# opendilab/LightZero

Hardware: NVIDIA H100
Metric: MCTS simulations/sec (batched search+infer) (higher is better)
Workload: dtype f32 (fp16x2-split tensor MMAs, fp32 accumulate)

## Files before the change

### lightzero_b200/csrc/conv_tc.cu

```cuda
#include <math.h>
#include <stdlib.h>
#include <string.h>

#include <algorithm>

#include "conv_tc.cuh"
#include "tc_ptx.cuh"

namespace lz {

constexpr int kCvConsumers = 256, kCvThreads = kCvConsumers + 32;
constexpr int kCvStages = 4;

struct CvBars {
    uint64_t full[kCvStages], empty[kCvStages];
    uint64_t in_full;
};

struct CvGeom {
    int nbands, rin, m_lo, mcount, NT, PR;
    size_t plane, part, phase, in_bytes, tap_bytes, smem;
};

__host__ __device__ inline CvGeom cv_geom(const ConvTc &p)
{
    CvGeom g;
    const int H = p.in.H, pitch = p.in.pitch, kg = p.in.C / 8;
    g.nbands = (H + p.band_h - 1) / p.band_h;
    g.rin = (p.band_h + 2) * pitch + 2;
    g.m_lo = pitch + 1;
    g.mcount = (p.G - 1) * g.rin + p.band_h * pitch;
    g.NT = (g.mcount + 127) / 128;
    g.PR = g.m_lo + g.NT * 128 + pitch + 2;
    if (g.PR < p.G * g.rin) g.PR = p.G * g.rin;
    g.plane = (size_t)g.PR * 16;
    g.part = (size_t)kg * g.plane;
    g.phase = 2 * g.part;
    g.in_bytes = (g.phase * p.in.nphase + 127) & ~(size_t)127;
    g.tap_bytes = (size_t)2 * kg * p.N * 16;
    g.smem = g.in_bytes + p.stages * g.tap_bytes + 1024;
    return g;
}

__device__ __forceinline__ void store_split2(unsigned char *hi_ptr, unsigned char *lo_ptr, float a, float b)
{
    a = fminf(fmaxf(a, -65504.0f), 65504.0f);
    b = fminf(fmaxf(b, -65504.0f), 65504.0f);
    const __half ha = __float2half_rn(a), hb = __float2half_rn(b);
    *reinterpret_cast<__half2 *>(hi_ptr) = __halves2half2(ha, hb);
    *reinterpret_cast<__half2 *>(lo_ptr) = __halves2half2(__float2half_rn(a - __half2float(ha)), __float2half_rn(b - __half2float(hb)));
}

template <int N>
__global__ void __launch_bounds__(kCvThreads, N == 128 ? 1 : 2) k_conv_tc(ConvTc p)
{
    extern __shared__ __align__(1024) unsigned char smem[];
    const CvGeom g = cv_geom(p);
    unsigned char *in_s = smem;
    unsigned char *ring = smem + g.in_bytes;
    CvBars *bars = reinterpret_cast<CvBars *>(ring + p.stages * g.tap_bytes);
    const int nstages = p.stages;
    const int tid = threadIdx.x, warp = __shfl_sync(0xffffffffu, tid >> 5, 0), lane = tid & 31;
    const int pitch = p.in.pitch, H = p.in.H, W = p.in.W, kg_in = p.in.C / 8;
    const int group = blockIdx.x / g.nbands, band = blockIdx.x - group * g.nbands;
    const int img0 = group * p.G, nimg = min(p.G, p.B - img0);
    const int y0 = band * p.band_h;
    const int rin0 = y0 * pitch - 1;
    const int npass = p.npass;

    if (tid == 0) {
        for (int i = 0; i < kCvStages; ++i) { mbar_init(&bars->full[i], 1); mbar_init(&bars->empty[i], kCvConsumers / 32); }
        mbar_init(&bars->in_full, 1);
        fence_mbar_init();
    }
    __syncthreads();

    if (warp == kCvConsumers / 32) {
        if (lane == 0) {
            const int grow0 = rin0 + 1;
            const int ncopy = min(g.rin, p.in.plane_rows - grow0);
            const uint32_t bytes = (uint32_t)ncopy * 16u;
            mbar_expect_tx(&bars->in_full, bytes * (uint32_t)(nimg * p.in.nphase * 2 * kg_in));
            for (int k = 0; k < nimg; ++k)
                for (int f = 0; f < p.in.nphase; ++f)
                    for (int part = 0; part < 2; ++part)
                        for (int kg = 0; kg < kg_in; ++kg) {
                            const unsigned char *src = p.in.base + (size_t)(img0 + k) * p.in.img_stride + f * p.in.phase_stride +
                                                       part * p.in.part_stride + ((size_t)kg * p.in.plane_rows + grow0) * 16;
                            unsigned char *dst = in_s + f * g.phase + part * g.part + kg * g.plane + (size_t)k * g.rin * 16;
                            bulk_g2s(dst, src, bytes, &bars->in_full);
                        }
            for (int n = 0; n < 9 * g.NT; ++n) {
                const int st = n % nstages, tap = n % 9;
                if (n >= nstages) mbar_wait(&bars->empty[st], ((n / nstages) - 1) & 1);
                mbar_expect_tx(&bars->full[st], (uint32_t)g.tap_bytes);
                bulk_g2s(ring + st * g.tap_bytes, p.w + (size_t)tap * g.tap_bytes, (uint32_t)g.tap_bytes, &bars->full[st]);
            }
        }
        return;
    }

    const int wg = warp >> 2;
    const uint32_t plane16 = (uint32_t)(g.plane >> 4);
    const uint64_t a_desc0 = make_desc(smem_u32(in_s), plane16, 8);
    const uint64_t b_desc0 = make_desc(smem_u32(ring), 2 * N, 8);
    const uint32_t b_lo16 = (uint32_t)N;
    const uint32_t a_lo16 = (uint32_t)(g.part >> 4);
    const int nks = kg_in / 2;
    const int yend = min(y0 + p.band_h, H);
    const int qc = 2 * (lane & 3);
    mbar_wait(&bars->in_full, 0);
    for (int t = 0; t < g.NT; ++t) {
        float acc[N / 2];
#pragma unroll
        for (int i = 0; i < N / 2; ++i) acc[i] = 0.0f;
        for (int tap = 0; tap < 9; ++tap) {
            const int n = t * 9 + tap, st = n % nstages;
            mbar_wait(&bars->full[st], (n / nstages) & 1);
            const uint64_t b0 = b_desc0 + (uint64_t)((st * g.tap_bytes) >> 4);
            const uint64_t a0 = a_desc0 + (uint64_t)((p.tap_phase[tap] * g.phase) >> 4) + (uint64_t)(g.m_lo + p.tap_shift[tap] + t * 128 + wg * 64);
            wg_fence();
            for (int ks = 0; ks < nks; ++ks) {
                wgmma_f16<N>(acc, a0 + ks * 2 * plane16, b0 + ks * 4 * N);
                if (npass == 3) {
                    wgmma_f16<N>(acc, a0 + ks * 2 * plane16, b0 + b_lo16 + ks * 4 * N);
                    wgmma_f16<N>(acc, a0 + a_lo16 + ks * 2 * plane16, b0 + ks * 4 * N);
                }
            }
            wg_commit();
            if (tap > 0) {
                wg_wait<1>();
                __syncwarp();
                if (lane == 0) mbar_arrive(&bars->empty[(n - 1) % nstages]);
            }
        }
        wg_wait<0>();
        __syncwarp();
        if (lane == 0) mbar_arrive(&bars->empty[(t * 9 + 8) % nstages]);

#pragma unroll
        for (int hr = 0; hr < 2; ++hr) {
            const int m = g.m_lo + t * 128 + wg * 64 + 16 * (warp & 3) + (lane >> 2) + 8 * hr;
            const int k = m / g.rin;
            const int rho = rin0 + (m - k * g.rin);
            const int yy = rho / pitch - 1, xx = rho - (yy + 1) * pitch;
            const bool in_band = (k < nimg) && (rho >= pitch) && (yy >= y0) && (yy < yend);
            const bool valid = in_band && (xx < W);
#pragma unroll
            for (int j = 0; j < N / 8; ++j) {
                const int col = 8 * j + qc;
                const int grp = (N == 128) ? (col >> 6) : 0;
                const int c = col - grp * 64;
                const Tcl &o = p.out[grp];
                const bool relu = p.relu[grp] != 0;
                float v0 = fmaf(acc[4 * j + 2 * hr], __ldg(p.scale + col), __ldg(p.shift + col));
                float v1 = fmaf(acc[4 * j + 2 * hr + 1], __ldg(p.scale + col + 1), __ldg(p.shift + col + 1));
                if (p.res.base && grp == 0 && valid) {
                    const unsigned char *rp = p.res.base + (size_t)(img0 + k) * p.res.img_stride +
                                              ((size_t)(c >> 3) * p.res.plane_rows + rho + 1) * 16 + (c & 7) * 2;
                    const float2 a = __half22float2(*reinterpret_cast<const __half2 *>(rp));
                    const float2 b = __half22float2(*reinterpret_cast<const __half2 *>(rp + p.res.part_stride));
                    v0 += a.x + b.x;
                    v1 += a.y + b.y;
                }
                v0 = valid ? (relu ? fmaxf(v0, 0.0f) : v0) : 0.0f;
                v1 = valid ? (relu ? fmaxf(v1, 0.0f) : v1) : 0.0f;
                if (in_band) {
                    unsigned char *op = o.base + (size_t)(img0 + k) * o.img_stride + ((size_t)(c >> 3) * o.plane_rows + rho + 1) * 16 + (c & 7) * 2;
                    store_split2(op, op + o.part_stride, v0, v1);
                }
            }
        }
    }
}

constexpr int kRbChunks = 16;

struct RbBars {
    uint64_t full[kCvStages], empty[kCvStages];
    uint64_t chunk[kRbChunks];
};

struct RbGeom {
    int nbands, S, m_lo, NT1, NT2, PR, nchunk;
    size_t plane, part, buf, tap_bytes, smem;
};

__host__ __device__ inline RbGeom rb_geom(const ResBlockTc &p)
{
    RbGeom g;
    const int H = p.in.H, pitch = p.in.pitch, kg = p.in.C / 8;
    g.nbands = (H + p.band_h - 1) / p.band_h;
    g.S = (p.band_h + 4) * pitch + 2;
    g.m_lo = pitch + 1;
    g.NT1 = ((p.G - 1) * g.S + (p.band_h + 2) * pitch + 127) / 128;
    g.NT2 = ((p.G - 1) * g.S + p.band_h * pitch + 127) / 128;
    g.PR = p.G * g.S;
    g.nchunk = (g.PR + 127) / 128;
    g.plane = (size_t)g.PR * 16;
    g.part = (size_t)kg * g.plane;
    g.buf = (2 * g.part + 127) & ~(size_t)127;
    g.tap_bytes = (size_t)2 * kg * p.in.C * 16;
    g.smem = 2 * g.buf + p.stages * g.tap_bytes + 1024;
    return g;
}

template <int N>
__device__ __forceinline__ void rb_tiles(float (&acc)[2][N / 2], bool two, uint64_t a_desc0, int row0, const ResBlockTc &p,
                                         const RbGeom &g, uint64_t b_desc0, RbBars *bars, int n0, int lane)
{
    const uint32_t plane16 = (uint32_t)(g.plane >> 4), a_lo16 = (uint32_t)(g.part >> 4), b_lo16 = (uint32_t)N;
    const int nstages = p.stages;
#pragma unroll
    for (int s = 0; s < 2; ++s)
#pragma unroll
        for (int i = 0; i < N / 2; ++i) acc[s][i] = 0.0f;
    for (int tap = 0; tap < 9; ++tap) {
        const int n = n0 + tap, st = n % nstages;
        mbar_wait(&bars->full[st], (n / nstages) & 1);
        const uint64_t b0 = b_desc0 + (uint64_t)((st * g.tap_bytes) >> 4);
        const uint64_t a0 = a_desc0 + (uint64_t)(row0 + p.tap_shift[tap]);
        wg_fence();
        for (int ks = 0; ks < N / 16; ++ks) {
#pragma unroll
            for (int s = 0; s < 2; ++s) {
                if (s == 1 && !two) break;
                const uint64_t as = a0 + s * 128 + ks * 2 * plane16;
                wgmma_f16<N>(acc[s], as, b0 + ks * 4 * N);
                if (p.npass == 3) {
                    wgmma_f16<N>(acc[s], as, b0 + b_lo16 + ks * 4 * N);
                    wgmma_f16<N>(acc[s], as + a_lo16, b0 + ks * 4 * N);
                }
            }
        }
        wg_commit();
        if (tap > 0) {
            wg_wait<1>();
            __syncwarp();
            if (lane == 0) mbar_arrive(&bars->empty[(n - 1) % nstages]);
        }
    }
    wg_wait<0>();
    __syncwarp();
    if (lane == 0) mbar_arrive(&bars->empty[(n0 + 8) % nstages]);
}

template <int N>
__global__ void __launch_bounds__(kCvThreads, 1) k_resblock_tc(ResBlockTc p)
{
    extern __shared__ __align__(1024) unsigned char smem[];
    const RbGeom g = rb_geom(p);
    unsigned char *in_s = smem, *mid_s = smem + g.buf, *ring = smem + 2 * g.buf;
    RbBars *bars = reinterpret_cast<RbBars *>(ring + p.stages * g.tap_bytes);
    const int nstages = p.stages;
    const int tid = threadIdx.x, warp = __shfl_sync(0xffffffffu, tid >> 5, 0), lane = tid & 31;
    const int pitch = p.in.pitch, H = p.in.H, W = p.in.W, kg_in = N / 8;
    const int group = blockIdx.x / g.nbands, band = blockIdx.x - group * g.nbands;
    const int img0 = group * p.G, nimg = min(p.G, p.B - img0);
    const int y0 = band * p.band_h;
    const int np1 = (g.NT1 + 1) / 2, ntaps = 9 * (np1 + (g.NT2 + 1) / 2);

    if (tid == 0) {
        for (int i = 0; i < kCvStages; ++i) { mbar_init(&bars->full[i], 1); mbar_init(&bars->empty[i], kCvConsumers / 32); }
        for (int c = 0; c < g.nchunk; ++c) mbar_init(&bars->chunk[c], 1);
        fence_mbar_init();
    }
    __syncthreads();

    if (warp == kCvConsumers / 32) {
        if (lane == 0) {
            auto load_tap = [&](int n) {
                const int st = n % nstages, tap = n % 9;
                if (n >= nstages) mbar_wait(&bars->empty[st], ((n / nstages) - 1) & 1);
                mbar_expect_tx(&bars->full[st], (uint32_t)g.tap_bytes);
                bulk_g2s(ring + st * g.tap_bytes, p.w[n >= 9 * np1] + (size_t)tap * g.tap_bytes, (uint32_t)g.tap_bytes, &bars->full[st]);
            };
            for (int n = 0; n < nstages; ++n) load_tap(n);
            const int g0 = (y0 - 1) * pitch;
            const int r0 = max(0, -g0), r1 = min(g.S, p.in.plane_rows - g0);
            for (int c = 0; c < g.nchunk; ++c) {
                uint32_t rows = 0;
                for (int k = 0; k < nimg; ++k) rows += (uint32_t)max(0, min(k * g.S + r1, c * 128 + 128) - max(k * g.S + r0, c * 128));
                mbar_expect_tx(&bars->chunk[c], rows * 16u * (uint32_t)(2 * kg_in));
                for (int k = 0; k < nimg; ++k) {
                    const int lo = max(k * g.S + r0, c * 128), hi = min(k * g.S + r1, c * 128 + 128);
                    if (hi <= lo) continue;
                    for (int part = 0; part < 2; ++part)
                        for (int kg = 0; kg < kg_in; ++kg) {
                            const unsigned char *src = p.in.base + (size_t)(img0 + k) * p.in.img_stride + part * p.in.part_stride +
                                                       ((size_t)kg * p.in.plane_rows + g0 + lo - k * g.S) * 16;
                            bulk_g2s(in_s + part * g.part + kg * g.plane + (size_t)lo * 16, src, (uint32_t)(hi - lo) * 16u, &bars->chunk[c]);
                        }
                }
            }
            for (int n = nstages; n < ntaps; ++n) load_tap(n);
        }
        return;
    }

    const int wg = warp >> 2;
    const uint32_t plane16 = (uint32_t)(g.plane >> 4);
    const uint64_t in_desc = make_desc(smem_u32(in_s), plane16, 8), mid_desc = make_desc(smem_u32(mid_s), plane16, 8);
    const uint64_t b_desc0 = make_desc(smem_u32(ring), 2 * N, 8);
    const int qc = 2 * (lane & 3);
    if (tid < 2 * kg_in) *reinterpret_cast<uint4 *>(mid_s + tid * g.plane) = make_uint4(0u, 0u, 0u, 0u);

    int ready = 0;
    for (int t = 0; t < g.NT1; t += 2) {
        const bool two = t + 1 < g.NT1;
        const int need = min(g.nchunk, (t * 128 + 256 + 2 * pitch + 1) / 128 + 1);
        for (; ready < need; ++ready) mbar_wait(&bars->chunk[ready], 0);
        float acc[2][N / 2];
        rb_tiles<N>(acc, two, in_desc, g.m_lo + t * 128 + wg * 64, p, g, b_desc0, bars, t / 2 * 9, lane);
#pragma unroll
        for (int e = 0; e < 4; ++e) {
            const int s = e >> 1, hr = e & 1;
            if (s == 1 && !two) break;
            const int m = g.m_lo + (t + s) * 128 + wg * 64 + 16 * (warp & 3) + (lane >> 2) + 8 * hr;
            const int i = m - pitch;
            const int k = m / g.S;
            const int rho = (y0 - 1) * pitch - 1 + (m - k * g.S);
            const int yy = rho / pitch - 1, xx = rho - (yy + 1) * pitch;
            const bool valid = (k < nimg) && (rho >= pitch) && (yy >= y0 - 1) && (yy <= y0 + p.band_h) && (yy < H) && (xx < W);
            if (i >= g.PR) continue;
#pragma unroll
            for (int j = 0; j < N / 8; ++j) {
                const int col = 8 * j + qc;
                float v0 = fmaf(acc[s][4 * j + 2 * hr], __ldg(p.scale[0] + col), __ldg(p.shift[0] + col));
                float v1 = fmaf(acc[s][4 * j + 2 * hr + 1], __ldg(p.scale[0] + col + 1), __ldg(p.shift[0] + col + 1));
                v0 = valid ? fmaxf(v0, 0.0f) : 0.0f;
                v1 = valid ? fmaxf(v1, 0.0f) : 0.0f;
                unsigned char *op = mid_s + (size_t)(col >> 3) * g.plane + (size_t)i * 16 + (col & 7) * 2;
                store_split2(op, op + g.part, v0, v1);
            }
        }
    }
    for (; ready < g.nchunk; ++ready) mbar_wait(&bars->chunk[ready], 0);
    fence_proxy_async();
    asm volatile("bar.sync 1, %0;\n" ::"n"(kCvConsumers) : "memory");

    const int yend = min(y0 + p.band_h, H);
    for (int t = 0; t < g.NT2; t += 2) {
        const bool two = t + 1 < g.NT2;
        float acc[2][N / 2];
        rb_tiles<N>(acc, two, mid_desc, g.m_lo + t * 128 + wg * 64, p, g, b_desc0, bars, (np1 + t / 2) * 9, lane);
#pragma unroll
        for (int e = 0; e < 4; ++e) {
            const int s = e >> 1, hr = e & 1;
            if (s == 1 && !two) break;
            const int m = g.m_lo + (t + s) * 128 + wg * 64 + 16 * (warp & 3) + (lane >> 2) + 8 * hr;
            const int k = m / g.S;
            const int rho = y0 * pitch - 1 + (m - k * g.S);
            const int yy = rho / pitch - 1, xx = rho - (yy + 1) * pitch;
            const bool in_band = (k < nimg) && (rho >= pitch) && (yy >= y0) && (yy < yend);
            const bool valid = in_band && (xx < W);
            const Tcl &o = p.out;
            size_t obase = 0;
            bool do_write = in_band;
            if (in_band) {
                if (o.nphase == 1) {
                    obase = (size_t)(img0 + k) * o.img_stride + (size_t)(rho + 1) * 16;
                } else if (valid) {
                    const int ph = (yy & 1) * 2 + (xx & 1);
                    const int rho2 = ((yy >> 1) + 1) * o.pitch + (xx >> 1);
                    obase = (size_t)(img0 + k) * o.img_stride + ph * o.phase_stride + (size_t)(rho2 + 1) * 16;
                } else {
                    do_write = false;
                }
            }
#pragma unroll
            for (int j = 0; j < N / 8; ++j) {
                const int col = 8 * j + qc;
                float v0 = fmaf(acc[s][4 * j + 2 * hr], __ldg(p.scale[1] + col), __ldg(p.shift[1] + col));
                float v1 = fmaf(acc[s][4 * j + 2 * hr + 1], __ldg(p.scale[1] + col + 1), __ldg(p.shift[1] + col + 1));
                if (valid) {
                    const unsigned char *rp = in_s + (size_t)(col >> 3) * g.plane + (size_t)(m + pitch) * 16 + (col & 7) * 2;
                    const float2 a = __half22float2(*reinterpret_cast<const __half2 *>(rp));
                    const float2 b = __half22float2(*reinterpret_cast<const __half2 *>(rp + g.part));
                    v0 += a.x + b.x;
                    v1 += a.y + b.y;
                }
                v0 = valid ? fmaxf(v0, 0.0f) : 0.0f;
                v1 = valid ? fmaxf(v1, 0.0f) : 0.0f;
                if (do_write) {
                    unsigned char *op = o.base + obase + (size_t)(col >> 3) * o.plane_rows * 16 + (col & 7) * 2;
                    store_split2(op, op + o.part_stride, v0, v1);
                }
            }
        }
    }
}

__device__ __forceinline__ void tcl_load8(const Tcl &t, int img, int kg, int rho, float (&v)[8])
{
    const unsigned char *pp = t.base + (size_t)img * t.img_stride + ((size_t)kg * t.plane_rows + rho + 1) * 16;
    const uint4 rh = __ldg(reinterpret_cast<const uint4 *>(pp));
    const uint4 rl = __ldg(reinterpret_cast<const uint4 *>(pp + t.part_stride));
    const __half2 *hh = reinterpret_cast<const __half2 *>(&rh), *hl = reinterpret_cast<const __half2 *>(&rl);
#pragma unroll
    for (int j = 0; j < 4; ++j) {
        const float2 a = __half22float2(hh[j]), b = __half22float2(hl[j]);
        v[2 * j] = a.x + b.x;
        v[2 * j + 1] = a.y + b.y;
    }
}

__global__ void k_pool_tcl(Tcl in, Tcl out, float *out_nchw, int B, int Hout)
{
    const int kgs = in.C / 8;
    const size_t n = (size_t)B * kgs * Hout * Hout;
    for (size_t i = blockIdx.x * (size_t)blockDim.x + threadIdx.x; i < n; i += (size_t)gridDim.x * blockDim.x) {
        const int xo = (int)(i % Hout), yo = (int)((i / Hout) % Hout);
        const int kg = (int)((i / ((size_t)Hout * Hout)) % kgs), img = (int)(i / ((size_t)Hout * Hout * kgs));
        float s[8];
#pragma unroll
        for (int j = 0; j < 8; ++j) s[j] = 0.0f;
#pragma unroll
        for (int ky = 0; ky < 3; ++ky) {
            const int yy = 2 * yo + ky - 1;
            if (yy < 0 || yy >= in.H) continue;
#pragma unroll
            for (int kx = 0; kx < 3; ++kx) {
                const int xx = 2 * xo + kx - 1;
                if (xx < 0 || xx >= in.W) continue;
                float v[8];
                tcl_load8(in, img, kg, (yy + 1) * in.pitch + xx, v);
#pragma unroll
                for (int j = 0; j < 8; ++j) s[j] += v[j];
            }
        }
#pragma unroll
        for (int j = 0; j < 8; ++j) s[j] = s[j] / 9.0f;
        if (out_nchw) {
#pragma unroll
            for (int j = 0; j < 8; ++j) out_nchw[((size_t)img * in.C + kg * 8 + j) * Hout * Hout + yo * Hout + xo] = s[j];
        } else {
            unsigned char *op = out.base + (size_t)img * out.img_stride + ((size_t)kg * out.plane_rows + (yo + 1) * out.pitch + xo + 1) * 16;
            store_split8(op, op + out.part_stride, s);
        }
    }
}

__global__ void k_tcl_to_nchw(Tcl in, float *out_nchw, int B)
{
    const int kgs = in.C / 8, H = in.H, W = in.W;
    const size_t n = (size_t)B * kgs * H * W;
    for (size_t i = blockIdx.x * (size_t)blockDim.x + threadIdx.x; i < n; i += (size_t)gridDim.x * blockDim.x) {
        const int x = (int)(i % W), y = (int)((i / W) % H);
        const int kg = (int)((i / ((size_t)W * H)) % kgs), img = (int)(i / ((size_t)W * H * kgs));
        float v[8];
        tcl_load8(in, img, kg, (y + 1) * in.pitch + x, v);
#pragma unroll
        for (int j = 0; j < 8; ++j) out_nchw[((size_t)img * in.C + kg * 8 + j) * H * W + y * W + x] = v[j];
    }
}

int conv_tc_prepare_launch()
{
    const int big = 227 * 1024;
    LZ_CUDA_CHECK(cudaFuncSetAttribute(k_conv_tc<64>, cudaFuncAttributeMaxDynamicSharedMemorySize, big));
    LZ_CUDA_CHECK(cudaFuncSetAttribute(k_conv_tc<128>, cudaFuncAttributeMaxDynamicSharedMemorySize, big));
    LZ_CUDA_CHECK(cudaFuncSetAttribute(k_resblock_tc<32>, cudaFuncAttributeMaxDynamicSharedMemorySize, big));
    LZ_CUDA_CHECK(cudaFuncSetAttribute(k_resblock_tc<64>, cudaFuncAttributeMaxDynamicSharedMemorySize, big));
    return LZ_OK;
}

int conv_tc_launch(const ConvTc &p, cudaStream_t s)
{
    const CvGeom g = cv_geom(p);
    LZ_REQUIRE(g.smem <= 227 * 1024, LZ_EINVAL, "conv_tc: band needs %zu B shared memory", g.smem);
    LZ_REQUIRE(g.tap_bytes <= 16384 && (p.in.C % 16) == 0, LZ_EINVAL, "conv_tc: unsupported channel counts");
    LZ_REQUIRE(p.out[0].nphase == 1 && (p.N < 128 || p.out[1].nphase == 1), LZ_EINVAL, "conv_tc: phase-split output is not supported");
    const int groups = (p.B + p.G - 1) / p.G;
    const int grid = groups * g.nbands;
    switch (p.N) {
        case 64: k_conv_tc<64><<<grid, kCvThreads, g.smem, s>>>(p); break;
        case 128: k_conv_tc<128><<<grid, kCvThreads, g.smem, s>>>(p); break;
        default: LZ_REQUIRE(false, LZ_EINVAL, "conv_tc: N must be 64 or 128");
    }
    LZ_KERNEL_CHECK();
    return LZ_OK;
}

int resblock_tc_plan(ResBlockTc &p)
{
    const int H = p.in.H, W = p.in.W;
    ResBlockTc q = p;
    double best = -1.0;
    for (int G = 1; G <= 4; ++G)
        for (int bh = (G > 1 ? H : 1); bh <= H; ++bh)
            for (int st = 2; st <= 4; st += 2) {
                q.G = G; q.band_h = bh; q.stages = st;
                const RbGeom g = rb_geom(q);
                if (g.smem > 227 * 1024 || g.nchunk > kRbChunks) continue;
                double score = (double)(2 * G * H * W) / ((double)g.nbands * (g.NT1 + g.NT2) * 128);
                score *= (st == 4) ? 1.0 : 0.97;
                if (score > best + 1e-9) { best = score; p.G = G; p.band_h = bh; p.stages = st; }
            }
    LZ_REQUIRE(best > 0.0, LZ_EINVAL, "resblock_tc: no band of a %dx%d, %d-channel block fits shared memory", H, W, p.in.C);
    return LZ_OK;
}

int resblock_tc_launch(const ResBlockTc &p, cudaStream_t s)
{
    const RbGeom g = rb_geom(p);
    LZ_REQUIRE(g.smem <= 227 * 1024 && g.nchunk <= kRbChunks, LZ_EINVAL, "resblock_tc: band needs %zu B shared memory", g.smem);
    LZ_REQUIRE(p.in.nphase == 1 && p.out.C == p.in.C, LZ_EINVAL, "resblock_tc: unsupported input / output layout");
    const int grid = (p.B + p.G - 1) / p.G * g.nbands;
    switch (p.in.C) {
        case 32: k_resblock_tc<32><<<grid, kCvThreads, g.smem, s>>>(p); break;
        case 64: k_resblock_tc<64><<<grid, kCvThreads, g.smem, s>>>(p); break;
        default: LZ_REQUIRE(false, LZ_EINVAL, "resblock_tc: channels must be 32 or 64");
    }
    LZ_KERNEL_CHECK();
    return LZ_OK;
}

size_t conv_tc_packed_bytes(int cin, int ncols) { return (size_t)9 * 2 * (cin / 8) * ncols * 16; }

float conv_tc_pack(const float *w, int cin, int cout, int ncols, int col0, unsigned char *dst)
{
    float mx = 0.0f;
    for (size_t i = 0; i < (size_t)cout * cin * 9; ++i) mx = std::max(mx, fabsf(w[i]));
    int e = 0;
    if (mx > 0.0f) frexpf(mx, &e);
    const float scale = ldexpf(1.0f, 13 - e);
    const size_t tap_halves = (size_t)2 * (cin / 8) * ncols * 8, part_halves = (size_t)ncols * 8;
    __half *h = reinterpret_cast<__half *>(dst);
    for (int t = 0; t < 9; ++t)
        for (int co = 0; co < cout; ++co)
            for (int ci = 0; ci < cin; ++ci) {
                const float sv = w[((size_t)co * cin + ci) * 9 + t] * scale;
                const __half hi = __float2half_rn(sv);
                const __half lo = __float2half_rn(sv - __half2float(hi));
                const size_t off = (size_t)t * tap_halves + ((size_t)(ci / 8) * 2 * ncols + col0 + co) * 8 + (ci % 8);
                h[off] = hi;
                h[off + part_halves] = lo;
            }
    return scale;
}

int pool_tcl_launch(const Tcl &in, const Tcl &out, int B, cudaStream_t s)
{
    const size_t n = (size_t)B * (in.C / 8) * out.H * out.W;
    k_pool_tcl<<<(int)std::min<size_t>((n + 255) / 256, kNumSMs * 32), 256, 0, s>>>(in, out, nullptr, B, out.H);
    LZ_KERNEL_CHECK();
    return LZ_OK;
}

int pool_tcl_to_nchw_launch(const Tcl &in, float *out, int B, int Hout, cudaStream_t s)
{
    const size_t n = (size_t)B * (in.C / 8) * Hout * Hout;
    Tcl dummy = in;
    k_pool_tcl<<<(int)std::min<size_t>((n + 255) / 256, kNumSMs * 32), 256, 0, s>>>(in, dummy, out, B, Hout);
    LZ_KERNEL_CHECK();
    return LZ_OK;
}

int tcl_to_nchw_launch(const Tcl &in, float *out, int B, cudaStream_t s)
{
    k_tcl_to_nchw<<<tcl_to_nchw_ctas(in, B), 256, 0, s>>>(in, out, B);
    LZ_KERNEL_CHECK();
    return LZ_OK;
}

int tcl_to_nchw_ctas(const Tcl &in, int B)
{
    const size_t n = (size_t)B * (in.C / 8) * in.H * in.W;
    return (int)std::min<size_t>((n + 255) / 256, kNumSMs * 32);
}

}
```

### lightzero_b200/csrc/tc_ptx.cuh

```cuda
#pragma once
#include <cuda_fp16.h>
#include <cuda_runtime.h>
#include <stdint.h>
#include <stdio.h>

namespace lz {

__device__ __forceinline__ uint32_t smem_u32(const void *p) { return (uint32_t)__cvta_generic_to_shared(p); }

__device__ __forceinline__ void mbar_init(uint64_t *bar, uint32_t count)
{
    asm volatile("mbarrier.init.shared::cta.b64 [%0], %1;\n" ::"r"(smem_u32(bar)), "r"(count));
}
__device__ __forceinline__ void mbar_arrive(uint64_t *bar)
{
    asm volatile("{\n\t.reg .b64 st;\n\tmbarrier.arrive.shared::cta.b64 st, [%0];\n\t}\n" ::"r"(smem_u32(bar)) : "memory");
}
__device__ __forceinline__ void mbar_expect_tx(uint64_t *bar, uint32_t bytes)
{
    asm volatile("{\n\t.reg .b64 st;\n\tmbarrier.arrive.expect_tx.shared::cta.b64 st, [%0], %1;\n\t}\n" ::"r"(smem_u32(bar)), "r"(bytes) : "memory");
}
__device__ __forceinline__ void mbar_wait(uint64_t *bar, uint32_t parity)
{
    const uint32_t a = smem_u32(bar);
    for (uint32_t it = 0; it < (1u << 28); ++it) {
        uint32_t ok;
        asm volatile("{\n\t.reg .pred p;\n\tmbarrier.try_wait.parity.shared::cta.b64 p, [%1], %2;\n\tselp.u32 %0, 1, 0, p;\n\t}\n"
                     : "=r"(ok) : "r"(a), "r"(parity) : "memory");
        if (ok) return;
    }
    asm volatile("trap;\n");
}
__device__ __forceinline__ void bulk_g2s(void *dst, const void *src, uint32_t bytes, uint64_t *bar)
{
    asm volatile("cp.async.bulk.shared::cluster.global.mbarrier::complete_tx::bytes [%0], [%1], %2, [%3];\n"
                 ::"r"(smem_u32(dst)), "l"(src), "r"(bytes), "r"(smem_u32(bar)) : "memory");
}
__device__ __forceinline__ void fence_proxy_async() { asm volatile("fence.proxy.async.shared::cta;\n" ::: "memory"); }
__device__ __forceinline__ void fence_mbar_init() { asm volatile("fence.mbarrier_init.release.cluster;\n" ::: "memory"); }

__device__ __forceinline__ void wg_fence() { asm volatile("wgmma.fence.sync.aligned;\n" ::: "memory"); }
__device__ __forceinline__ void wg_commit() { asm volatile("wgmma.commit_group.sync.aligned;\n" ::: "memory"); }
template <int N>
__device__ __forceinline__ void wg_wait() { asm volatile("wgmma.wait_group.sync.aligned %0;\n" ::"n"(N) : "memory"); }

template <int N>
__device__ __forceinline__ void wg_fence_acc(float (&d)[N])
{
#pragma unroll
    for (int i = 0; i < N; ++i) asm volatile("" : "+f"(d[i])::"memory");
}

#define LZ_WG_R8(o) "+f"(d[o + 0]), "+f"(d[o + 1]), "+f"(d[o + 2]), "+f"(d[o + 3]), "+f"(d[o + 4]), "+f"(d[o + 5]), "+f"(d[o + 6]), "+f"(d[o + 7])
__device__ __forceinline__ void wgmma_n16(float (&d)[8], uint64_t a, uint64_t b)
{
    asm volatile("{\n\t.reg .pred p;\n\tsetp.ne.b32 p, 1, 0;\n\t"
                 "wgmma.mma_async.sync.aligned.m64n16k16.f32.f16.f16 {%0, %1, %2, %3, %4, %5, %6, %7}, %8, %9, p, 1, 1, 0, 0;\n\t}\n"
                 : LZ_WG_R8(0) : "l"(a), "l"(b));
}
__device__ __forceinline__ void wgmma_n32(float (&d)[16], uint64_t a, uint64_t b)
{
    asm volatile("{\n\t.reg .pred p;\n\tsetp.ne.b32 p, 1, 0;\n\t"
                 "wgmma.mma_async.sync.aligned.m64n32k16.f32.f16.f16 {%0, %1, %2, %3, %4, %5, %6, %7, %8, %9, %10, %11, %12, %13, %14, "
                 "%15}, %16, %17, p, 1, 1, 0, 0;\n\t}\n"
                 : LZ_WG_R8(0), LZ_WG_R8(8) : "l"(a), "l"(b));
}
__device__ __forceinline__ void wgmma_n64(float (&d)[32], uint64_t a, uint64_t b)
{
    asm volatile("{\n\t.reg .pred p;\n\tsetp.ne.b32 p, 1, 0;\n\t"
                 "wgmma.mma_async.sync.aligned.m64n64k16.f32.f16.f16 {%0, %1, %2, %3, %4, %5, %6, %7, %8, %9, %10, %11, %12, %13, %14, "
                 "%15, %16, %17, %18, %19, %20, %21, %22, %23, %24, %25, %26, %27, %28, %29, %30, %31}, %32, %33, p, 1, 1, 0, 0;\n\t}\n"
                 : LZ_WG_R8(0), LZ_WG_R8(8), LZ_WG_R8(16), LZ_WG_R8(24) : "l"(a), "l"(b));
}
__device__ __forceinline__ void wgmma_n128(float (&d)[64], uint64_t a, uint64_t b)
{
    asm volatile("{\n\t.reg .pred p;\n\tsetp.ne.b32 p, 1, 0;\n\t"
                 "wgmma.mma_async.sync.aligned.m64n128k16.f32.f16.f16 {%0, %1, %2, %3, %4, %5, %6, %7, %8, %9, %10, %11, %12, %13, %14, "
                 "%15, %16, %17, %18, %19, %20, %21, %22, %23, %24, %25, %26, %27, %28, %29, %30, %31, %32, %33, %34, %35, %36, %37, %38, "
                 "%39, %40, %41, %42, %43, %44, %45, %46, %47, %48, %49, %50, %51, %52, %53, %54, %55, %56, %57, %58, %59, %60, %61, %62, "
                 "%63}, %64, %65, p, 1, 1, 0, 0;\n\t}\n"
                 : LZ_WG_R8(0), LZ_WG_R8(8), LZ_WG_R8(16), LZ_WG_R8(24), LZ_WG_R8(32), LZ_WG_R8(40), LZ_WG_R8(48), LZ_WG_R8(56)
                 : "l"(a), "l"(b));
}
#undef LZ_WG_R8
template <int N>
__device__ __forceinline__ void wgmma_f16(float (&d)[N / 2], uint64_t a, uint64_t b)
{
    if constexpr (N == 16) wgmma_n16(d, a, b);
    else if constexpr (N == 32) wgmma_n32(d, a, b);
    else if constexpr (N == 64) wgmma_n64(d, a, b);
    else wgmma_n128(d, a, b);
}

template <int N>
__device__ __forceinline__ void wg_stage(float *S, int ld, int row0, int col0, const float (&d)[N / 2])
{
    const int w = (threadIdx.x >> 5) & 3, lane = threadIdx.x & 31;
    float *p0 = S + (size_t)(row0 + 16 * w + (lane >> 2)) * ld + col0 + 2 * (lane & 3), *p1 = p0 + 8 * ld;
#pragma unroll
    for (int j = 0; j < N / 8; ++j) {
        *reinterpret_cast<float2 *>(p0 + 8 * j) = make_float2(d[4 * j], d[4 * j + 1]);
        *reinterpret_cast<float2 *>(p1 + 8 * j) = make_float2(d[4 * j + 2], d[4 * j + 3]);
    }
}

__device__ __forceinline__ uint64_t make_desc(uint32_t saddr, uint32_t lbo16, uint32_t sbo16)
{
    return (uint64_t)((saddr >> 4) & 0x3FFFu) | ((uint64_t)(lbo16 & 0x3FFFu) << 16) | ((uint64_t)(sbo16 & 0x3FFFu) << 32);
}

__device__ __forceinline__ void store_split8(unsigned char *hi_ptr, unsigned char *lo_ptr, const float *v)
{
    __half2 h[4], l[4];
#pragma unroll
    for (int i = 0; i < 4; ++i) {
        float a = v[2 * i], b = v[2 * i + 1];
        a = fminf(fmaxf(a, -65504.0f), 65504.0f);
        b = fminf(fmaxf(b, -65504.0f), 65504.0f);
        __half ha = __float2half_rn(a), hb = __float2half_rn(b);
        h[i] = __halves2half2(ha, hb);
        l[i] = __halves2half2(__float2half_rn(a - __half2float(ha)), __float2half_rn(b - __half2float(hb)));
    }
    *reinterpret_cast<uint4 *>(hi_ptr) = *reinterpret_cast<uint4 *>(h);
    *reinterpret_cast<uint4 *>(lo_ptr) = *reinterpret_cast<uint4 *>(l);
}


__device__ __forceinline__ void store_split8_pos(unsigned char *hi_ptr, unsigned char *lo_ptr, const float *v)
{
    __half2 h[4], l[4];
#pragma unroll
    for (int i = 0; i < 4; ++i) {
        const float a = fminf(v[2 * i], 65504.0f), b = fminf(v[2 * i + 1], 65504.0f);
        h[i] = __floats2half2_rn(a, b);
        const float2 back = __half22float2(h[i]);
        l[i] = __floats2half2_rn(a - back.x, b - back.y);
    }
    *reinterpret_cast<uint4 *>(hi_ptr) = *reinterpret_cast<uint4 *>(h);
    *reinterpret_cast<uint4 *>(lo_ptr) = *reinterpret_cast<uint4 *>(l);
}

}
```

Baseline: 5.054 million.

## Fold hi*lo and lo*hi split MMAs into one wide wgmma; enlarge resblock tile groups

For the 3-pass fp16 split, the hi-A×lo-B and hi-A×hi-B products are issued as a single double-width wgmma (B hi/lo halves laid out contiguously), leaving one extra N-wide MMA for lo-A. This cuts wgmma issue count and keeps the A reuse, then sums the two accumulator halves in the epilogue. The resblock kernel also groups up to 6 tiles for C=32, adds a full producer warpgroup and uses setmaxnreg to move registers to consumers. The risks are higher register pressure and spills from the doubled accumulators, and reliance on the B layout where the lo part sits at offset N.

Measured after the change: 5.203 million (median of 6 runs). 2.9% higher.

```diff
diff --git a/lightzero_b200/csrc/conv_tc.cu b/lightzero_b200/csrc/conv_tc.cu
--- a/lightzero_b200/csrc/conv_tc.cu
+++ b/lightzero_b200/csrc/conv_tc.cu
@@ -51,6 +51,13 @@
     *reinterpret_cast<__half2 *>(lo_ptr) = __halves2half2(__float2half_rn(a - __half2float(ha)), __float2half_rn(b - __half2float(hb)));
 }
 
+template <bool Fold, int K>
+__device__ __forceinline__ float fold_sum(const float (&acc)[K], int r, int npass)
+{
+    if constexpr (Fold) return npass == 3 ? acc[r] + acc[K / 2 + r] : acc[r];
+    else return acc[r];
+}
+
 template <int N>
 __global__ void __launch_bounds__(kCvThreads, N == 128 ? 1 : 2) k_conv_tc(ConvTc p)
 {
@@ -67,6 +74,8 @@
     const int y0 = band * p.band_h;
     const int rin0 = y0 * pitch - 1;
     const int npass = p.npass;
+    constexpr bool kFold = N <= 64;
+    constexpr int kFoldN = kFold ? N : N / 2;
 
     if (tid == 0) {
         for (int i = 0; i < kCvStages; ++i) { mbar_init(&bars->full[i], 1); mbar_init(&bars->empty[i], kCvConsumers / 32); }
@@ -111,9 +120,10 @@
     const int qc = 2 * (lane & 3);
     mbar_wait(&bars->in_full, 0);
     for (int t = 0; t < g.NT; ++t) {
-        float acc[N / 2];
-#pragma unroll
-        for (int i = 0; i < N / 2; ++i) acc[i] = 0.0f;
+        float acc[kFoldN];
+#pragma unroll
+        for (int i = 0; i < kFoldN; ++i) acc[i] = 0.0f;
+        float (&acc_hi)[N / 2] = *reinterpret_cast<float (*)[N / 2]>(acc);
         for (int tap = 0; tap < 9; ++tap) {
             const int n = t * 9 + tap, st = n % nstages;
             mbar_wait(&bars->full[st], (n / nstages) & 1);
@@ -121,10 +131,16 @@
             const uint64_t a0 = a_desc0 + (uint64_t)((p.tap_phase[tap] * g.phase) >> 4) + (uint64_t)(g.m_lo + p.tap_shift[tap] + t * 128 + wg * 64);
             wg_fence();
             for (int ks = 0; ks < nks; ++ks) {
-                wgmma_f16<N>(acc, a0 + ks * 2 * plane16, b0 + ks * 4 * N);
-                if (npass == 3) {
-                    wgmma_f16<N>(acc, a0 + ks * 2 * plane16, b0 + b_lo16 + ks * 4 * N);
-                    wgmma_f16<N>(acc, a0 + a_lo16 + ks * 2 * plane16, b0 + ks * 4 * N);
+                const uint64_t as = a0 + ks * 2 * plane16, bs = b0 + ks * 4 * N;
+                if (npass != 3) {
+                    wgmma_f16<N>(acc_hi, as, bs);
+                } else if constexpr (kFold) {
+                    wgmma_f16<2 * N>(acc, as, bs);
+                    wgmma_f16<N>(acc_hi, as + a_lo16, bs);
+                } else {
+                    wgmma_f16<N>(acc, as, bs);
+                    wgmma_f16<N>(acc, as, bs + b_lo16);
+                    wgmma_f16<N>(acc, as + a_lo16, bs);
                 }
             }
             wg_commit();
@@ -153,8 +169,9 @@
                 const int c = col - grp * 64;
                 const Tcl &o = p.out[grp];
                 const bool relu = p.relu[grp] != 0;
-                float v0 = fmaf(acc[4 * j + 2 * hr], __ldg(p.scale + col), __ldg(p.shift + col));
-                float v1 = fmaf(acc[4 * j + 2 * hr + 1], __ldg(p.scale + col + 1), __ldg(p.shift + col + 1));
+                const int r = 4 * j + 2 * hr;
+                float v0 = fmaf(fold_sum<kFold>(acc, r, npass), __ldg(p.scale + col), __ldg(p.shift + col));
+                float v1 = fmaf(fold_sum<kFold>(acc, r + 1, npass), __ldg(p.scale + col + 1), __ldg(p.shift + col + 1));
                 if (p.res.base && grp == 0 && valid) {
                     const unsigned char *rp = p.res.base + (size_t)(img0 + k) * p.res.img_stride +
                                               ((size_t)(c >> 3) * p.res.plane_rows + rho + 1) * 16 + (c & 7) * 2;
@@ -175,6 +192,8 @@
 }
 
 constexpr int kRbChunks = 16;
+constexpr int kRbThreads = kCvConsumers + 128;
+constexpr int kRbProducerRegs = 40, kRbConsumerRegs = 232;
 
 struct RbBars {
     uint64_t full[kCvStages], empty[kCvStages];
@@ -206,15 +225,18 @@
 }
 
 template <int N>
-__device__ __forceinline__ void rb_tiles(float (&acc)[2][N / 2], bool two, uint64_t a_desc0, int row0, const ResBlockTc &p,
+__host__ __device__ constexpr int rb_group_tiles() { return N == 32 ? 6 : 2; }
+
+template <int N, int T>
+__device__ __forceinline__ void rb_tiles(float (&acc)[T][N], int ntile, uint64_t a_desc0, int row0, const ResBlockTc &p,
                                          const RbGeom &g, uint64_t b_desc0, RbBars *bars, int n0, int lane)
 {
-    const uint32_t plane16 = (uint32_t)(g.plane >> 4), a_lo16 = (uint32_t)(g.part >> 4), b_lo16 = (uint32_t)N;
+    const uint32_t plane16 = (uint32_t)(g.plane >> 4), a_lo16 = (uint32_t)(g.part >> 4);
     const int nstages = p.stages;
 #pragma unroll
-    for (int s = 0; s < 2; ++s)
-#pragma unroll
-        for (int i = 0; i < N / 2; ++i) acc[s][i] = 0.0f;
+    for (int s = 0; s < T; ++s)
+#pragma unroll
+        for (int i = 0; i < N; ++i) acc[s][i] = 0.0f;
     for (int tap = 0; tap < 9; ++tap) {
         const int n = n0 + tap, st = n % nstages;
         mbar_wait(&bars->full[st], (n / nstages) & 1);
@@ -223,13 +245,15 @@
         wg_fence();
         for (int ks = 0; ks < N / 16; ++ks) {
 #pragma unroll
-            for (int s = 0; s < 2; ++s) {
-                if (s == 1 && !two) break;
-                const uint64_t as = a0 + s * 128 + ks * 2 * plane16;
-                wgmma_f16<N>(acc[s], as, b0 + ks * 4 * N);
+            for (int s = 0; s < T; ++s) {
+                if (s >= ntile) break;
+                const uint64_t as = a0 + s * 128 + ks * 2 * plane16, bs = b0 + ks * 4 * N;
+                float (&acc_hi)[N / 2] = *reinterpret_cast<float (*)[N / 2]>(acc[s]);
                 if (p.npass == 3) {
-                    wgmma_f16<N>(acc[s], as, b0 + b_lo16 + ks * 4 * N);
-                    wgmma_f16<N>(acc[s], as + a_lo16, b0 + ks * 4 * N);
+                    wgmma_f16<2 * N>(acc[s], as, bs);
+                    wgmma_f16<N>(acc_hi, as + a_lo16, bs);
+                } else {
+                    wgmma_f16<N>(acc_hi, as, bs);
                 }
             }
         }
@@ -246,7 +270,7 @@
 }
 
 template <int N>
-__global__ void __launch_bounds__(kCvThreads, 1) k_resblock_tc(ResBlockTc p)
+__global__ void __launch_bounds__(kRbThreads, 1) k_resblock_tc(ResBlockTc p)
 {
     extern __shared__ __align__(1024) unsigned char smem[];
     const RbGeom g = rb_geom(p);
@@ -258,7 +282,8 @@
     const int group = blockIdx.x / g.nbands, band = blockIdx.x - group * g.nbands;
     const int img0 = group * p.G, nimg = min(p.G, p.B - img0);
     const int y0 = band * p.band_h;
-    const int np1 = (g.NT1 + 1) / 2, ntaps = 9 * (np1 + (g.NT2 + 1) / 2);
+    constexpr int T = rb_group_tiles<N>();
+    const int np1 = (g.NT1 + T - 1) / T, ntaps = 9 * (np1 + (g.NT2 + T - 1) / T);
 
     if (tid == 0) {
         for (int i = 0; i < kCvStages; ++i) { mbar_init(&bars->full[i], 1); mbar_init(&bars->empty[i], kCvConsumers / 32); }
@@ -267,8 +292,9 @@
     }
     __syncthreads();
 
-    if (warp == kCvConsumers / 32) {
-        if (lane == 0) {
+    if (warp >= kCvConsumers / 32) {
+        setmaxnreg_dec<kRbProducerRegs>();
+        if (warp == kCvConsumers / 32 && lane == 0) {
             auto load_tap = [&](int n) {
                 const int st = n % nstages, tap = n % 9;
                 if (n >= nstages) mbar_wait(&bars->empty[st], ((n / nstages) - 1) & 1);
@@ -298,6 +324,7 @@
         return;
     }
 
+    setmaxnreg_inc<kRbConsumerRegs>();
     const int wg = warp >> 2;
     const uint32_t plane16 = (uint32_t)(g.plane >> 4);
     const uint64_t in_desc = make_desc(smem_u32(in_s), plane16, 8), mid_desc = make_desc(smem_u32(mid_s), plane16, 8);
@@ -306,16 +333,16 @@
     if (tid < 2 * kg_in) *reinterpret_cast<uint4 *>(mid_s + tid * g.plane) = make_uint4(0u, 0u, 0u, 0u);
 
     int ready = 0;
-    for (int t = 0; t < g.NT1; t += 2) {
-        const bool two = t + 1 < g.NT1;
-        const int need = min(g.nchunk, (t * 128 + 256 + 2 * pitch + 1) / 128 + 1);
+    for (int t = 0; t < g.NT1; t += T) {
+        const int ntile = min(T, g.NT1 - t);
+        const int need = min(g.nchunk, (t * 128 + 128 * T + 2 * pitch + 1) / 128 + 1);
         for (; ready < need; ++ready) mbar_wait(&bars->chunk[ready], 0);
-        float acc[2][N / 2];
-        rb_tiles<N>(acc, two, in_desc, g.m_lo + t * 128 + wg * 64, p, g, b_desc0, bars, t / 2 * 9, lane);
-#pragma unroll
-        for (int e = 0; e < 4; ++e) {
+        float acc[T][N];
+        rb_tiles<N, T>(acc, ntile, in_desc, g.m_lo + t * 128 + wg * 64, p, g, b_desc0, bars, t / T * 9, lane);
+#pragma unroll
+        for (int e = 0; e < 2 * T; ++e) {
             const int s = e >> 1, hr = e & 1;
-            if (s == 1 && !two) break;
+            if (s >= ntile) break;
             const int m = g.m_lo + (t + s) * 128 + wg * 64 + 16 * (warp & 3) + (lane >> 2) + 8 * hr;
             const int i = m - pitch;
             const int k = m / g.S;
@@ -326,8 +353,9 @@
 #pragma unroll
             for (int j = 0; j < N / 8; ++j) {
                 const int col = 8 * j + qc;
-                float v0 = fmaf(acc[s][4 * j + 2 * hr], __ldg(p.scale[0] + col), __ldg(p.shift[0] + col));
-                float v1 = fmaf(acc[s][4 * j + 2 * hr + 1], __ldg(p.scale[0] + col + 1), __ldg(p.shift[0] + col + 1));
+                const int r = 4 * j + 2 * hr;
+                float v0 = fmaf(fold_sum<true>(acc[s], r, p.npass), __ldg(p.scale[0] + col), __ldg(p.shift[0] + col));
+                float v1 = fmaf(fold_sum<true>(acc[s], r + 1, p.npass), __ldg(p.scale[0] + col + 1), __ldg(p.shift[0] + col + 1));
                 v0 = valid ? fmaxf(v0, 0.0f) : 0.0f;
                 v1 = valid ? fmaxf(v1, 0.0f) : 0.0f;
                 unsigned char *op = mid_s + (size_t)(col >> 3) * g.plane + (size_t)i * 16 + (col & 7) * 2;
@@ -340,14 +368,14 @@
     asm volatile("bar.sync 1, %0;\n" ::"n"(kCvConsumers) : "memory");
 
     const int yend = min(y0 + p.band_h, H);
-    for (int t = 0; t < g.NT2; t += 2) {
-        const bool two = t + 1 < g.NT2;
-        float acc[2][N / 2];
-        rb_tiles<N>(acc, two, mid_desc, g.m_lo + t * 128 + wg * 64, p, g, b_desc0, bars, (np1 + t / 2) * 9, lane);
-#pragma unroll
-        for (int e = 0; e < 4; ++e) {
+    for (int t = 0; t < g.NT2; t += T) {
+        const int ntile = min(T, g.NT2 - t);
+        float acc[T][N];
+        rb_tiles<N, T>(acc, ntile, mid_desc, g.m_lo + t * 128 + wg * 64, p, g, b_desc0, bars, (np1 + t / T) * 9, lane);
+#pragma unroll
+        for (int e = 0; e < 2 * T; ++e) {
             const int s = e >> 1, hr = e & 1;
-            if (s == 1 && !two) break;
+            if (s >= ntile) break;
             const int m = g.m_lo + (t + s) * 128 + wg * 64 + 16 * (warp & 3) + (lane >> 2) + 8 * hr;
             const int k = m / g.S;
             const int rho = y0 * pitch - 1 + (m - k * g.S);
@@ -371,8 +399,9 @@
 #pragma unroll
             for (int j = 0; j < N / 8; ++j) {
                 const int col = 8 * j + qc;
-                float v0 = fmaf(acc[s][4 * j + 2 * hr], __ldg(p.scale[1] + col), __ldg(p.shift[1] + col));
-                float v1 = fmaf(acc[s][4 * j + 2 * hr + 1], __ldg(p.scale[1] + col + 1), __ldg(p.shift[1] + col + 1));
+                const int r = 4 * j + 2 * hr;
+                float v0 = fmaf(fold_sum<true>(acc[s], r, p.npass), __ldg(p.scale[1] + col), __ldg(p.shift[1] + col));
+                float v1 = fmaf(fold_sum<true>(acc[s], r + 1, p.npass), __ldg(p.scale[1] + col + 1), __ldg(p.shift[1] + col + 1));
                 if (valid) {
                     const unsigned char *rp = in_s + (size_t)(col >> 3) * g.plane + (size_t)(m + pitch) * 16 + (col & 7) * 2;
                     const float2 a = __half22float2(*reinterpret_cast<const __half2 *>(rp));
@@ -508,8 +537,8 @@
     LZ_REQUIRE(p.in.nphase == 1 && p.out.C == p.in.C, LZ_EINVAL, "resblock_tc: unsupported input / output layout");
     const int grid = (p.B + p.G - 1) / p.G * g.nbands;
     switch (p.in.C) {
-        case 32: k_resblock_tc<32><<<grid, kCvThreads, g.smem, s>>>(p); break;
-        case 64: k_resblock_tc<64><<<grid, kCvThreads, g.smem, s>>>(p); break;
+        case 32: k_resblock_tc<32><<<grid, kRbThreads, g.smem, s>>>(p); break;
+        case 64: k_resblock_tc<64><<<grid, kRbThreads, g.smem, s>>>(p); break;
         default: LZ_REQUIRE(false, LZ_EINVAL, "resblock_tc: channels must be 32 or 64");
     }
     LZ_KERNEL_CHECK();
diff --git a/lightzero_b200/csrc/tc_ptx.cuh b/lightzero_b200/csrc/tc_ptx.cuh
--- a/lightzero_b200/csrc/tc_ptx.cuh
+++ b/lightzero_b200/csrc/tc_ptx.cuh
@@ -43,6 +43,11 @@
 __device__ __forceinline__ void wg_commit() { asm volatile("wgmma.commit_group.sync.aligned;\n" ::: "memory"); }
 template <int N>
 __device__ __forceinline__ void wg_wait() { asm volatile("wgmma.wait_group.sync.aligned %0;\n" ::"n"(N) : "memory"); }
+
+template <int R>
+__device__ __forceinline__ void setmaxnreg_inc() { asm volatile("setmaxnreg.inc.sync.aligned.u32 %0;\n" ::"n"(R)); }
+template <int R>
+__device__ __forceinline__ void setmaxnreg_dec() { asm volatile("setmaxnreg.dec.sync.aligned.u32 %0;\n" ::"n"(R)); }
 
 template <int N>
 __device__ __forceinline__ void wg_fence_acc(float (&d)[N])
```

## Generalize tensor-core tile grouping to amortize weight-tap loads across more M tiles

Applied to the files above, without the earlier changes.

Moves the per-tap wgmma loop into a shared tc_group helper that processes a configurable number of 128-row M tiles per weight-tap pass. The resblock kernel raises this from 2 to 6 tiles for N=32, and spreads tiles evenly across groups, so each tap weight load is reused by more tiles and fewer tap stages are streamed. Chunk readiness waits become per tile rather than per pair. The plain conv kernel keeps one tile per group. The cost is higher register pressure from six accumulator arrays, which risks spills or lower occupancy.

Measured after the change: 5.040 million before, 5.228 million after (median of 6 runs). 1.04x the previous value.

```diff
diff --git a/lightzero_b200/csrc/conv_tc.cu b/lightzero_b200/csrc/conv_tc.cu
--- a/lightzero_b200/csrc/conv_tc.cu
+++ b/lightzero_b200/csrc/conv_tc.cu
@@ -51,6 +51,63 @@
     *reinterpret_cast<__half2 *>(lo_ptr) = __halves2half2(__float2half_rn(a - __half2float(ha)), __float2half_rn(b - __half2float(hb)));
 }
 
+__host__ __device__ inline void tile_groups(int NT, int MT, int &ng, int &per)
+{
+    ng = (NT + MT - 1) / MT;
+    per = (NT + ng - 1) / ng;
+}
+
+template <int N, int MT, int KS, typename TapA, typename TileReady>
+__device__ __forceinline__ void tc_group(float (&acc)[MT][N / 2], int nt, TapA tap_a, TileReady tile_ready, int nks, int npass,
+                                         uint32_t plane16, uint32_t a_lo16, uint64_t b_desc0, size_t tap_bytes, int nstages,
+                                         uint64_t *full, uint64_t *empty, int n0, int lane)
+{
+    const uint32_t b_lo16 = (uint32_t)N;
+#pragma unroll
+    for (int s = 0; s < MT; ++s)
+#pragma unroll
+        for (int i = 0; i < N / 2; ++i) acc[s][i] = 0.0f;
+    for (int tap = 0; tap < 9; ++tap) {
+        const int n = n0 + tap, st = n % nstages;
+        mbar_wait(&full[st], (n / nstages) & 1);
+        const uint64_t b0 = b_desc0 + (uint64_t)((st * tap_bytes) >> 4);
+        const uint64_t a0 = tap_a(tap);
+        auto kstep = [&](int ks) {
+#pragma unroll
+            for (int s = 0; s < MT; ++s) {
+                if (s >= nt) break;
+                if (tap == 0 && ks == 0) tile_ready(s);
+                const uint64_t as = a0 + s * 128 + ks * 2 * plane16;
+                wgmma_f16<N>(acc[s], as, b0 + ks * 4 * N);
+                if (npass == 3) {
+                    wgmma_f16<N>(acc[s], as, b0 + b_lo16 + ks * 4 * N);
+                    wgmma_f16<N>(acc[s], as + a_lo16, b0 + ks * 4 * N);
+                }
+            }
+        };
+        wg_fence();
+        if constexpr (KS > 0) {
+#pragma unroll
+            for (int ks = 0; ks < KS; ++ks) kstep(ks);
+        } else {
+#pragma unroll 1
+            for (int ks = 0; ks < nks; ++ks) kstep(ks);
+        }
+        wg_commit();
+        if (tap > 0) {
+            wg_wait<1>();
+            __syncwarp();
+            if (lane == 0) mbar_arrive(&empty[(n - 1) % nstages]);
+        }
+    }
+    wg_wait<0>();
+    __syncwarp();
+    if (lane == 0) mbar_arrive(&empty[(n0 + 8) % nstages]);
+}
+
+template <int N>
+constexpr int kCvTiles = 1;
+
 template <int N>
 __global__ void __launch_bounds__(kCvThreads, N == 128 ? 1 : 2) k_conv_tc(ConvTc p)
 {
@@ -66,7 +123,9 @@
     const int img0 = group * p.G, nimg = min(p.G, p.B - img0);
     const int y0 = band * p.band_h;
     const int rin0 = y0 * pitch - 1;
-    const int npass = p.npass;
+    constexpr int MT = kCvTiles<N>;
+    int ng, per;
+    tile_groups(g.NT, MT, ng, per);
 
     if (tid == 0) {
         for (int i = 0; i < kCvStages; ++i) { mbar_init(&bars->full[i], 1); mbar_init(&bars->empty[i], kCvConsumers / 32); }
@@ -90,7 +149,7 @@
                             unsigned char *dst = in_s + f * g.phase + part * g.part + kg * g.plane + (size_t)k * g.rin * 16;
                             bulk_g2s(dst, src, bytes, &bars->in_full);
                         }
-            for (int n = 0; n < 9 * g.NT; ++n) {
+            for (int n = 0; n < 9 * ng; ++n) {
                 const int st = n % nstages, tap = n % 9;
                 if (n >= nstages) mbar_wait(&bars->empty[st], ((n / nstages) - 1) & 1);
                 mbar_expect_tx(&bars->full[st], (uint32_t)g.tap_bytes);
@@ -104,43 +163,24 @@
     const uint32_t plane16 = (uint32_t)(g.plane >> 4);
     const uint64_t a_desc0 = make_desc(smem_u32(in_s), plane16, 8);
     const uint64_t b_desc0 = make_desc(smem_u32(ring), 2 * N, 8);
-    const uint32_t b_lo16 = (uint32_t)N;
     const uint32_t a_lo16 = (uint32_t)(g.part >> 4);
-    const int nks = kg_in / 2;
     const int yend = min(y0 + p.band_h, H);
     const int qc = 2 * (lane & 3);
     mbar_wait(&bars->in_full, 0);
-    for (int t = 0; t < g.NT; ++t) {
-        float acc[N / 2];
-#pragma unroll
-        for (int i = 0; i < N / 2; ++i) acc[i] = 0.0f;
-        for (int tap = 0; tap < 9; ++tap) {
-            const int n = t * 9 + tap, st = n % nstages;
-            mbar_wait(&bars->full[st], (n / nstages) & 1);
-            const uint64_t b0 = b_desc0 + (uint64_t)((st * g.tap_bytes) >> 4);
-            const uint64_t a0 = a_desc0 + (uint64_t)((p.tap_phase[tap] * g.phase) >> 4) + (uint64_t)(g.m_lo + p.tap_shift[tap] + t * 128 + wg * 64);
-            wg_fence();
-            for (int ks = 0; ks < nks; ++ks) {
-                wgmma_f16<N>(acc, a0 + ks * 2 * plane16, b0 + ks * 4 * N);
-                if (npass == 3) {
-                    wgmma_f16<N>(acc, a0 + ks * 2 * plane16, b0 + b_lo16 + ks * 4 * N);
-                    wgmma_f16<N>(acc, a0 + a_lo16 + ks * 2 * plane16, b0 + ks * 4 * N);
-                }
-            }
-            wg_commit();
-            if (tap > 0) {
-                wg_wait<1>();
-                __syncwarp();
-                if (lane == 0) mbar_arrive(&bars->empty[(n - 1) % nstages]);
-            }
-        }
-        wg_wait<0>();
-        __syncwarp();
-        if (lane == 0) mbar_arrive(&bars->empty[(t * 9 + 8) % nstages]);
-
-#pragma unroll
-        for (int hr = 0; hr < 2; ++hr) {
-            const int m = g.m_lo + t * 128 + wg * 64 + 16 * (warp & 3) + (lane >> 2) + 8 * hr;
+    for (int gi = 0; gi < ng; ++gi) {
+        const int t0 = gi * per, nt = min(per, g.NT - t0);
+        float acc[MT][N / 2];
+        auto tap_a = [&](int tap) {
+            return a_desc0 + (uint64_t)((p.tap_phase[tap] * g.phase) >> 4) + (uint64_t)(g.m_lo + p.tap_shift[tap] + t0 * 128 + wg * 64);
+        };
+        tc_group<N, MT, 0>(acc, nt, tap_a, [](int) {}, kg_in / 2, p.npass, plane16, a_lo16, b_desc0, g.tap_bytes, nstages, bars->full,
+                           bars->empty, gi * 9, lane);
+
+#pragma unroll
+        for (int e = 0; e < 2 * MT; ++e) {
+            const int s = e >> 1, hr = e & 1;
+            if (s >= nt) break;
+            const int m = g.m_lo + (t0 + s) * 128 + wg * 64 + 16 * (warp & 3) + (lane >> 2) + 8 * hr;
             const int k = m / g.rin;
             const int rho = rin0 + (m - k * g.rin);
             const int yy = rho / pitch - 1, xx = rho - (yy + 1) * pitch;
@@ -153,8 +193,8 @@
                 const int c = col - grp * 64;
                 const Tcl &o = p.out[grp];
                 const bool relu = p.relu[grp] != 0;
-                float v0 = fmaf(acc[4 * j + 2 * hr], __ldg(p.scale + col), __ldg(p.shift + col));
-                float v1 = fmaf(acc[4 * j + 2 * hr + 1], __ldg(p.scale + col + 1), __ldg(p.shift + col + 1));
+                float v0 = fmaf(acc[s][4 * j + 2 * hr], __ldg(p.scale + col), __ldg(p.shift + col));
+                float v1 = fmaf(acc[s][4 * j + 2 * hr + 1], __ldg(p.scale + col + 1), __ldg(p.shift + col + 1));
                 if (p.res.base && grp == 0 && valid) {
                     const unsigned char *rp = p.res.base + (size_t)(img0 + k) * p.res.img_stride +
                                               ((size_t)(c >> 3) * p.res.plane_rows + rho + 1) * 16 + (c & 7) * 2;
@@ -206,44 +246,7 @@
 }
 
 template <int N>
-__device__ __forceinline__ void rb_tiles(float (&acc)[2][N / 2], bool two, uint64_t a_desc0, int row0, const ResBlockTc &p,
-                                         const RbGeom &g, uint64_t b_desc0, RbBars *bars, int n0, int lane)
-{
-    const uint32_t plane16 = (uint32_t)(g.plane >> 4), a_lo16 = (uint32_t)(g.part >> 4), b_lo16 = (uint32_t)N;
-    const int nstages = p.stages;
-#pragma unroll
-    for (int s = 0; s < 2; ++s)
-#pragma unroll
-        for (int i = 0; i < N / 2; ++i) acc[s][i] = 0.0f;
-    for (int tap = 0; tap < 9; ++tap) {
-        const int n = n0 + tap, st = n % nstages;
-        mbar_wait(&bars->full[st], (n / nstages) & 1);
-        const uint64_t b0 = b_desc0 + (uint64_t)((st * g.tap_bytes) >> 4);
-        const uint64_t a0 = a_desc0 + (uint64_t)(row0 + p.tap_shift[tap]);
-        wg_fence();
-        for (int ks = 0; ks < N / 16; ++ks) {
-#pragma unroll
-            for (int s = 0; s < 2; ++s) {
-                if (s == 1 && !two) break;
-                const uint64_t as = a0 + s * 128 + ks * 2 * plane16;
-                wgmma_f16<N>(acc[s], as, b0 + ks * 4 * N);
-                if (p.npass == 3) {
-                    wgmma_f16<N>(acc[s], as, b0 + b_lo16 + ks * 4 * N);
-                    wgmma_f16<N>(acc[s], as + a_lo16, b0 + ks * 4 * N);
-                }
-            }
-        }
-        wg_commit();
-        if (tap > 0) {
-            wg_wait<1>();
-            __syncwarp();
-            if (lane == 0) mbar_arrive(&bars->empty[(n - 1) % nstages]);
-        }
-    }
-    wg_wait<0>();
-    __syncwarp();
-    if (lane == 0) mbar_arrive(&bars->empty[(n0 + 8) % nstages]);
-}
+constexpr int kRbTiles = N == 32 ? 6 : 2;
 
 template <int N>
 __global__ void __launch_bounds__(kCvThreads, 1) k_resblock_tc(ResBlockTc p)
@@ -258,7 +261,11 @@
     const int group = blockIdx.x / g.nbands, band = blockIdx.x - group * g.nbands;
     const int img0 = group * p.G, nimg = min(p.G, p.B - img0);
     const int y0 = band * p.band_h;
-    const int np1 = (g.NT1 + 1) / 2, ntaps = 9 * (np1 + (g.NT2 + 1) / 2);
+    constexpr int MT = kRbTiles<N>;
+    int ng1, per1, ng2, per2;
+    tile_groups(g.NT1, MT, ng1, per1);
+    tile_groups(g.NT2, MT, ng2, per2);
+    const int ntaps = 9 * (ng1 + ng2);
 
     if (tid == 0) {
         for (int i = 0; i < kCvStages; ++i) { mbar_init(&bars->full[i], 1); mbar_init(&bars->empty[i], kCvConsumers / 32); }
@@ -273,7 +280,7 @@
                 const int st = n % nstages, tap = n % 9;
                 if (n >= nstages) mbar_wait(&bars->empty[st], ((n / nstages) - 1) & 1);
                 mbar_expect_tx(&bars->full[st], (uint32_t)g.tap_bytes);
-                bulk_g2s(ring + st * g.tap_bytes, p.w[n >= 9 * np1] + (size_t)tap * g.tap_bytes, (uint32_t)g.tap_bytes, &bars->full[st]);
+                bulk_g2s(ring + st * g.tap_bytes, p.w[n >= 9 * ng1] + (size_t)tap * g.tap_bytes, (uint32_t)g.tap_bytes, &bars->full[st]);
             };
             for (int n = 0; n < nstages; ++n) load_tap(n);
             const int g0 = (y0 - 1) * pitch;
@@ -302,21 +309,26 @@
     const uint32_t plane16 = (uint32_t)(g.plane >> 4);
     const uint64_t in_desc = make_desc(smem_u32(in_s), plane16, 8), mid_desc = make_desc(smem_u32(mid_s), plane16, 8);
     const uint64_t b_desc0 = make_desc(smem_u32(ring), 2 * N, 8);
+    const uint32_t a_lo16 = (uint32_t)(g.part >> 4);
     const int qc = 2 * (lane & 3);
     if (tid < 2 * kg_in) *reinterpret_cast<uint4 *>(mid_s + tid * g.plane) = make_uint4(0u, 0u, 0u, 0u);
 
     int ready = 0;
-    for (int t = 0; t < g.NT1; t += 2) {
-        const bool two = t + 1 < g.NT1;
-        const int need = min(g.nchunk, (t * 128 + 256 + 2 * pitch + 1) / 128 + 1);
-        for (; ready < need; ++ready) mbar_wait(&bars->chunk[ready], 0);
-        float acc[2][N / 2];
-        rb_tiles<N>(acc, two, in_desc, g.m_lo + t * 128 + wg * 64, p, g, b_desc0, bars, t / 2 * 9, lane);
-#pragma unroll
-        for (int e = 0; e < 4; ++e) {
+    for (int gi = 0; gi < ng1; ++gi) {
+        const int t0 = gi * per1, nt = min(per1, g.NT1 - t0);
+        float acc[MT][N / 2];
+        auto tap_a = [&](int tap) { return in_desc + (uint64_t)(g.m_lo + t0 * 128 + wg * 64 + p.tap_shift[tap]); };
+        auto tile_ready = [&](int s) {
+            const int need = min(g.nchunk, ((t0 + s) * 128 + 128 + 2 * pitch + 1) / 128 + 1);
+            for (; ready < need; ++ready) mbar_wait(&bars->chunk[ready], 0);
+        };
+        tc_group<N, MT, N / 16>(acc, nt, tap_a, tile_ready, N / 16, p.npass, plane16, a_lo16, b_desc0, g.tap_bytes, nstages, bars->full,
+                                bars->empty, gi * 9, lane);
+#pragma unroll
+        for (int e = 0; e < 2 * MT; ++e) {
             const int s = e >> 1, hr = e & 1;
-            if (s == 1 && !two) break;
-            const int m = g.m_lo + (t + s) * 128 + wg * 64 + 16 * (warp & 3) + (lane >> 2) + 8 * hr;
+            if (s >= nt) break;
+            const int m = g.m_lo + (t0 + s) * 128 + wg * 64 + 16 * (warp & 3) + (lane >> 2) + 8 * hr;
             const int i = m - pitch;
             const int k = m / g.S;
             const int rho = (y0 - 1) * pitch - 1 + (m - k * g.S);
@@ -340,15 +352,17 @@
     asm volatile("bar.sync 1, %0;\n" ::"n"(kCvConsumers) : "memory");
 
     const int yend = min(y0 + p.band_h, H);
-    for (int t = 0; t < g.NT2; t += 2) {
-        const bool two = t + 1 < g.NT2;
-        float acc[2][N / 2];
-        rb_tiles<N>(acc, two, mid_desc, g.m_lo + t * 128 + wg * 64, p, g, b_desc0, bars, (np1 + t / 2) * 9, lane);
-#pragma unroll
-        for (int e = 0; e < 4; ++e) {
+    for (int gi = 0; gi < ng2; ++gi) {
+        const int t0 = gi * per2, nt = min(per2, g.NT2 - t0);
+        float acc[MT][N / 2];
+        auto tap_a = [&](int tap) { return mid_desc + (uint64_t)(g.m_lo + t0 * 128 + wg * 64 + p.tap_shift[tap]); };
+        tc_group<N, MT, N / 16>(acc, nt, tap_a, [](int) {}, N / 16, p.npass, plane16, a_lo16, b_desc0, g.tap_bytes, nstages, bars->full,
+                                bars->empty, (ng1 + gi) * 9, lane);
+#pragma unroll
+        for (int e = 0; e < 2 * MT; ++e) {
             const int s = e >> 1, hr = e & 1;
-            if (s == 1 && !two) break;
-            const int m = g.m_lo + (t + s) * 128 + wg * 64 + 16 * (warp & 3) + (lane >> 2) + 8 * hr;
+            if (s >= nt) break;
+            const int m = g.m_lo + (t0 + s) * 128 + wg * 64 + 16 * (warp & 3) + (lane >> 2) + 8 * hr;
             const int k = m / g.S;
             const int rho = y0 * pitch - 1 + (m - k * g.S);
             const int yy = rho / pitch - 1, xx = rho - (yy + 1) * pitch;
```
